# Quyans/SG-NeRF

Measured on AMD Instinct MI355X. Metric: rays/sec + ms/frame, 800×800×64 samples, ScanNet scene, 1/2/4/8 GPU, higher is better.
Workload: dtype f32 (3xf16 split MFMA, fp32 accumulate); 1 GPU; synth-room 800x800 rays x SR=64 samples, D=400, K=8, P=26, 1200000 neural points (BASELINE config 2, 1 frame per rank per step); rays_per_frame=640000, SR=64, K=8, D=400, points=1200000, parallelism=frame-sharded x1, outputs=rgb, ray mask, background transmission, coarse_point_opacity [R, SR]

## Files before the change

### sg-nerf_amd/csrc/mlp_x3.hip

```cpp
#include <cstdio>
#include <cstdlib>
#include <algorithm>
#include <cmath>
#include <utility>
#include <vector>

#include "agg_device.h"
#include "x3_split.h"

namespace sgn {
namespace {
namespace x3 {

constexpr int NW16 = 8, TPB16 = NW16 * 64;
constexpr int PAIR = 2048;
constexpr int NSLOT = 2;
constexpr int PD = 2;
constexpr size_t PROJ_BYTES_PER_POINT = HID * 4;
struct XL {
    int ks, tp, np, kc;
    uint32_t off;
};
__host__ __device__ constexpr int nch(XL l) { return (l.ks + l.kc - 1) / l.kc; }
__host__ __device__ constexpr int nk(XL l, int c) { return l.ks - c * l.kc < l.kc ? l.ks - c * l.kc : l.kc; }

template <class Net>
struct Sched {
    static constexpr int layer_chunks(int l) { return Net::L[l].np * nch(Net::L[l]); }
    static constexpr int base(int l) { return l == 0 ? 0 : base(l - 1) + layer_chunks(l - 1); }
    static constexpr int total() { return base(Net::NL); }
    static constexpr int idx(int l, int p, int c) { return base(l) + p * nch(Net::L[l]) + c; }
    static constexpr int cl(int n, int l = 0) { return (l + 1 >= Net::NL || n < base(l + 1)) ? l : cl(n, l + 1); }
    static constexpr int cp(int n) { return (n - base(cl(n))) / nch(Net::L[cl(n)]); }
    static constexpr int cc(int n) { return (n - base(cl(n))) % nch(Net::L[cl(n)]); }
    static constexpr uint32_t off(int n) {
        return Net::L[cl(n)].off +
               (uint32_t)((cp(n) * Net::L[cl(n)].ks + cc(n) * Net::L[cl(n)].kc) * Net::L[cl(n)].tp) * PAIR;
    }
    static constexpr int pairs(int n) { return nk(Net::L[cl(n)], cc(n)) * Net::L[cl(n)].tp; }
};

__device__ __forceinline__ X3Pair lrelu_split8(const float (&a)[8], float inv) {
    float v[8];
#pragma unroll
    for (int j = 0; j < 8; ++j) v[j] = lrelu_x3(a[j] * inv);
    return split8_unit(v);
}

__device__ __forceinline__ void lds_dma_1k(const WBlob &wb, char *dst, int w, int lane, uint32_t soff) {
    asm volatile("" : "+s"(soff));
    __builtin_amdgcn_raw_ptr_buffer_load_lds(wb.rsrc, (__attribute__((address_space(3))) void *)(dst + w * 1024), 16,
                                             lane * 16 + w * 1024, soff, 0, 0);
}

template <class Net, int N, int NWv = NW16>
__device__ __forceinline__ void dma_chunk(const WBlob &wb, char *dst, int w, int lane) {
    using S = Sched<Net>;
    constexpr int nf = 2 * S::pairs(N);
    static_for<(nf + NWv - 1) / NWv>([&](auto jj) {
        constexpr int J = decltype(jj)::value;
        const int i = w + NWv * J;
        if (NWv * (J + 1) <= nf || i < nf)
            lds_dma_1k(wb, dst + NWv * J * 1024, w, lane, S::off(N) + (uint32_t)(NWv * J * 1024));
    });
}

template <class Net, int N, int J, int NWv = NW16>
__device__ __forceinline__ void dma_piece(const WBlob &wb, char *dst, int w, int lane) {
    using S = Sched<Net>;
    constexpr int nf = 2 * S::pairs(N);
    constexpr int PW = (nf + NWv - 1) / NWv;
    const int i = w * PW + J;
    if (nf % NWv == 0 || i < nf) {
        uint32_t soff = S::off(N) + (uint32_t)((J & ~3) * 1024);
        asm volatile("" : "+s"(soff));
        __builtin_amdgcn_raw_ptr_buffer_load_lds(wb.rsrc,
                                                 (__attribute__((address_space(3))) void *)(dst + (w * PW + (J & ~3)) * 1024),
                                                 16, lane * 16 + w * PW * 1024, soff, (J & 3) * 1024, 0);
    }
}
template <class Net, int N, int NWv = NW16>
constexpr int dma_pieces() { return (2 * Sched<Net>::pairs(N) + NWv - 1) / NWv; }

template <int VM = 0>
__device__ __forceinline__ void chunk_enter() {
    static_assert(VM >= 0 && VM < 64, "vmcnt range");
    if constexpr (VM == 0)
        asm volatile("s_waitcnt vmcnt(0)" ::: "memory");
    else
        __builtin_amdgcn_s_waitcnt((VM & 15) | (7 << 4) | (15 << 8) | ((VM >> 4) << 14));
    asm volatile("s_waitcnt lgkmcnt(0)" ::: "memory");
    __builtin_amdgcn_s_barrier();
}

struct NoHook {
    template <class C>
    __device__ void operator()(C) const {}
};
struct VmZero {
    static constexpr int vm(int) { return 0; }
};

constexpr uint32_t OFF16_W0B = 0;
constexpr uint32_t OFF16_W1 = OFF16_W0B + 32 * PAIR;
constexpr uint32_t OFF16_W2 = OFF16_W1 + 128 * PAIR;
constexpr uint32_t OFF16_W3 = OFF16_W2 + 144 * PAIR;
constexpr uint32_t OFF16_W0A = OFF16_W3 + 128 * PAIR;
constexpr uint32_t OFF16_WB = OFF16_W0A + 112 * PAIR;
constexpr uint32_t OFF16_C0 = OFF16_WB + 176 * PAIR;
constexpr uint32_t OFF16_C1 = OFF16_C0 + 72 * PAIR;
constexpr uint32_t OFF16_C2 = OFF16_C1 + 32 * PAIR;
constexpr uint32_t OFF16_F32 = OFF16_C2 + 32 * PAIR;
constexpr int Y_B0 = 0, Y_B1 = 256, Y_B2 = 512, Y_B3 = 768, Y_WA = 1024, Y_BB = 1280, Y_BA = 1536, Y_INV = 1537;
constexpr int Y_CB0 = Y_INV + 8 + 3, Y_CB1 = Y_CB0 + 128, Y_CB2 = Y_CB1 + 128, Y_CW3 = Y_CB2 + 128, Y_CB3 = Y_CW3 + 384;
constexpr int N_Y32 = Y_CB3 + 4;
constexpr size_t BLOB_BYTES_ALL = OFF16_F32 + (size_t)N_Y32 * 4;
__host__ __device__ constexpr size_t blob_bytes_sg(int) { return BLOB_BYTES_ALL; }
static_assert(N_Y32 % 4 == 0, "fp32 section in 16-B units");

constexpr int NWR = 4;
struct NetR16T {
    static constexpr int NW = NWR, SP = 16;
    static constexpr int KC = SP / 16;
    static constexpr int NL = 4;
    static constexpr XL L[NL] = {{2, 16, 1, KC, OFF16_W0B}, {8, 16, 1, KC, OFF16_W1}, {9, 16, 1, KC, OFF16_W2},
                                 {8, 8, 2, 2 * KC, OFF16_W3}};
};
template <int KB>
struct NetR16SGT {
    static constexpr int NW = NetR16T::NW, SP = NetR16T::SP, KC = NetR16T::KC;
    static constexpr int NL = 5;
    static constexpr XL L[NL] = {{2, 16, 1, KC, OFF16_W0B}, {8, 16, 1, KC, OFF16_W1}, {KB, 16, 1, KC, OFF16_WB},
                                 {9, 16, 1, KC, OFF16_W2}, {8, 8, 2, 2 * KC, OFF16_W3}};
};
struct NetProj16 {
    static constexpr int NW = NW16, SP = 32;
    static constexpr int NL = 1;
    static constexpr XL L[NL] = {{7, 16, 1, 2, OFF16_W0A}};
};
constexpr int NWC = 8, SPC = 32, KCC = SPC / 8;
struct NetColor16 {
    static constexpr int NW = NWC, SP = SPC;
    static constexpr int NL = 3;
    static constexpr XL L[NL] = {{9, 8, 1, KCC, OFF16_C0}, {4, 8, 1, KCC, OFF16_C1}, {4, 8, 1, KCC, OFF16_C2}};
};
static_assert(Sched<NetR16T>::total() == 27, "16x16 row stream");
static_assert(Sched<NetColor16>::total() == 5 && Sched<NetColor16>::pairs(2) == 8, "16x16 colour stream");

__device__ __forceinline__ f32x4 mfma16(h8 a, h8 b, f32x4 c) {
    return __builtin_amdgcn_mfma_f32_16x16x32_f16(a, b, c, 0, 0, 0);
}

template <int NS>
struct X3S {
    X3Pair b[NS];
};

template <class Net, int L, bool TRANS = false, class Vm = VmZero, int P = 0, int AOFF = 0, bool PIPE = false,
          int NS, int NA, class InFn, class PostFn = NoHook, class EndFn = NoHook, class MidFn = NoHook>
__device__ __forceinline__ void run_layer_ns(const WBlob &wb, char *lds, int &slot, int w, int lane,
                                             f32x4 (&acc)[NS][NA], InFn &&in, PostFn &&post = PostFn{},
                                             EndFn &&end = EndFn{}, MidFn &&mid = MidFn{}) {
    constexpr XL ly = Net::L[L];
    constexpr int TP = ly.tp;
    static_assert((TP == 16 || TP == 8) && P < ly.np, "passes of 16 or 8 output tiles");
    static_assert(AOFF + TP <= NA, "accumulator view");
    X3S<NS> Bn;
    if constexpr (PIPE) Bn = in(std::integral_constant<int, 0>{});
    static_for<nch(ly)>([&](auto cc) {
        constexpr int C = decltype(cc)::value;
        constexpr int N = Sched<Net>::idx(L, P, C), NN = (N + 1) % Sched<Net>::total();
        constexpr int NWv = Net::NW, SLOTv = Net::SP * PAIR;
        static_assert(nk(ly, C) * TP <= Net::SP, "chunk larger than a ring slot");
        chunk_enter<Vm::vm(C)>();
        post(cc);
        const char *sl = lds + slot * SLOTv;
        char *dnext = lds + (slot ^ 1) * SLOTv;
        constexpr int NF = nk(ly, C) * TP;
        constexpr int PW = dma_pieces<Net, NN, NWv>();
        auto frag = [&](int f, int part) { return *(const h8 *)(sl + (2 * f + part) * 1024 + lane * 16); };
        h8 fh[PD], fl[PD];
#pragma unroll
        for (int f = 0; f < PD; ++f) {
            fh[f] = frag(f, 0);
            fl[f] = frag(f, 1);
        }
        __builtin_amdgcn_sched_group_barrier(0x100, 2 * PD, 0);
        static_for<nk(ly, C)>([&](auto kk) {
            constexpr int KK = decltype(kk)::value;
            constexpr int KS = C * ly.kc + KK;
            if constexpr (NS > 1 && KK > 0 && !PIPE) __builtin_amdgcn_sched_barrier(0);
            X3S<NS> B;
            if constexpr (PIPE) B = Bn;
            else B = in(std::integral_constant<int, KS>{});
            static_for<TP>([&](auto tt) {
                constexpr int t = decltype(tt)::value, F = KK * TP + t;
                const h8 Ah = fh[F % PD], Al = fl[F % PD];
                if constexpr (F + PD < NF) {
                    fh[F % PD] = frag(F + PD, 0);
                    fl[F % PD] = frag(F + PD, 1);
                }
#pragma unroll
                for (int s = 0; s < NS; ++s) {
                    f32x4 &c = acc[s][AOFF + t];
                    if constexpr (TRANS) {
                        c = mfma16(B.b[s].hi, Al, c);
                        c = mfma16(B.b[s].lo, Ah, c);
                        c = mfma16(B.b[s].hi, Ah, c);
                    } else {
                        c = mfma16(Al, B.b[s].hi, c);
                        c = mfma16(Ah, B.b[s].lo, c);
                        c = mfma16(Ah, B.b[s].hi, c);
                    }
                }
                constexpr int NSP = NF / 2 > 0 ? NF / 2 : 1;
                if constexpr (F < NSP) {
                    static_for<(F + 1) * PW / NSP - F * PW / NSP>([&](auto jj) {
                        dma_piece<Net, NN, F * PW / NSP + decltype(jj)::value, NWv>(wb, dnext, w, lane);
                    });
                }
                mid(std::integral_constant<int, (C * ly.kc + KK) * TP + t>{});
                if constexpr (PIPE && t == TP / 2 - 1 && KS + 1 < ly.ks)
                    Bn = in(std::integral_constant<int, (KS + 1 < ly.ks ? KS + 1 : KS)>{});
                if constexpr (NS == 1) {
                    __builtin_amdgcn_sched_group_barrier(0x008, 1, 0);
                    __builtin_amdgcn_sched_group_barrier(0x100, 1, 0);
                    __builtin_amdgcn_sched_group_barrier(0x008, 1, 0);
                    __builtin_amdgcn_sched_group_barrier(0x100, 1, 0);
                    __builtin_amdgcn_sched_group_barrier(0x008, 1, 0);
                } else {
                    __builtin_amdgcn_sched_group_barrier(0x008, 3 * NS / 2, 0);
                    __builtin_amdgcn_sched_group_barrier(0x100, 1, 0);
                    __builtin_amdgcn_sched_group_barrier(0x008, 3 * NS - 3 * NS / 2, 0);
                    __builtin_amdgcn_sched_group_barrier(0x100, 1, 0);
                }
            });
        });
        __builtin_amdgcn_sched_barrier(0);
        end(cc);
        slot ^= 1;
        __builtin_amdgcn_sched_barrier(0);
    });
}

template <class Net, int L, bool TRANS = false, class Vm = VmZero, int P = 0, class InFn,
          class PostFn = NoHook, class EndFn = NoHook, class MidFn = NoHook>
__device__ __forceinline__ void run_layer16(const WBlob &wb, char *lds, int &slot, int w, int lane,
                                            f32x4 (&acc)[Net::L[L].tp], InFn &&in, PostFn &&post = PostFn{},
                                            EndFn &&end = EndFn{}, MidFn &&mid = MidFn{}) {
    constexpr int TP = Net::L[L].tp;
    run_layer_ns<Net, L, TRANS, Vm, P, 0>(wb, lds, slot, w, lane, reinterpret_cast<f32x4(&)[1][TP]>(acc),
                                          [&](auto k) { return X3S<1>{{in(k)}}; }, post, end, mid);
}

struct Proj16Args {
    const float *emb;
    int64_t n;
    const void *blob;
    float *proj;
    const float *xyz, *color, *dir, *conf;
    float *rec;
    const int32_t *idx;
    const int64_t *n_dev;
};
constexpr int REC16_FLOATS = 16;
constexpr int Y_LDS_OFF = NSLOT * NetProj16::SP * PAIR;
constexpr int PROJ16_LDS = Y_LDS_OFF + N_Y32 * 4;

__global__ __launch_bounds__(TPB16, 1) void k_point_proj16(Proj16Args a) {
    __shared__ __attribute__((aligned(16))) char lds[PROJ16_LDS];
    const int lane = threadIdx.x & 63, g = lane >> 4;
    const int w = __builtin_amdgcn_readfirstlane(threadIdx.x >> 6);
    const WBlob wb = make_blob(a.blob, BLOB_BYTES_ALL);
    {
        const float *src = (const float *)((const char *)a.blob + OFF16_F32);
        float *dst = (float *)(lds + Y_LDS_OFF);
        for (int i = threadIdx.x; i < N_Y32; i += TPB16) dst[i] = src[i];
    }
    __syncthreads();
    int slot = 0;
    dma_chunk<NetProj16, 0, NW16>(wb, lds, w, lane);
    const int64_t n = a.idx ? min(*a.n_dev, a.n) : a.n;
    const int64_t ntile = (n + 16 * NW16 - 1) / (16 * NW16);
    for (int64_t tile = blockIdx.x; tile < ntile; tile += gridDim.x) {
        int lz = 0;
        asm volatile("" : "+s"(lz));
        const float *Yl = (const float *)(lds + lz + Y_LDS_OFF);
        const int64_t j = tile * (16 * NW16) + w * 16 + (lane & 15);
        const bool ok = j < n;
        const int64_t p = a.idx ? (ok ? (int64_t)a.idx[j] : 0) : j;
        float f8[8];
        {
            const f32x4 *e4 = (const f32x4 *)(a.emb + (ok ? p : 0) * 32 + 8 * g);
            const f32x4 u0 = e4[0], u1 = e4[1];
            f8[0] = u0[0]; f8[1] = u0[1]; f8[2] = u0[2]; f8[3] = u0[3];
            f8[4] = u1[0]; f8[5] = u1[1]; f8[6] = u1[2]; f8[7] = u1[3];
        }
        f32x4 acc[16];
#pragma unroll
        for (int t = 0; t < 16; ++t) acc[t] = *(const f32x4 *)(Yl + Y_B0 + 16 * t + 4 * g);
        auto in = [&](auto k) {
            constexpr int S = decltype(k)::value;
            float v[8];
            if constexpr (S == 0) {
#pragma unroll
                for (int j = 0; j < 8; ++j) v[j] = f8[j];
            } else {
                static_for<4>([&](auto jp) {
                    constexpr int q = 8 * (S - 1) + 2 * decltype(jp)::value, dl = q / 6, f = (q % 6) / 2;
                    float sv, cv;
                    sincos_f<f>(f8[dl], sv, cv);
                    v[2 * decltype(jp)::value] = sv;
                    v[2 * decltype(jp)::value + 1] = cv;
                });
            }
            return split8_unit(v);
        };
        f32x4 q{};
        {
            const float *src = g == 0 ? a.xyz : g == 1 ? a.color : a.dir;
            const int64_t pc = ok ? p : 0;
            if (g < 3) q = f32x4{src[pc * 3], src[pc * 3 + 1], src[pc * 3 + 2], g == 0 ? a.conf[pc] : 0.f};
        }
        run_layer16<NetProj16, 0>(wb, lds + lz, slot, w, lane, acc, in);
        if (ok) {
            float *dst = a.proj + p * HID + 4 * g;
#pragma unroll
            for (int t = 0; t < 16; ++t) *(f32x4 *)(dst + 16 * t) = acc[t];
            *(f32x4 *)(a.rec + p * REC16_FLOATS + 4 * g) = q;
        }
    }
    asm volatile("s_waitcnt vmcnt(0)" ::: "memory");
}

constexpr int WG16_SAMPLES = NWR * 2;
constexpr int TPBR = NWR * 64;
constexpr int YR_OFF = NSLOT * NetR16T::SP * PAIR;
constexpr int YT16_OFF = YR_OFF + N_Y32 * 4;
constexpr int ROWS16_LDS = YT16_OFF + 2 * 16 * 20 * 4;
static_assert(2 * ROWS16_LDS <= 163840, "LDS budget (16x16 rows, two workgroups per CU)");

template <bool PERS, bool ROT = false>
struct Rec16 {
    float p[3], col[3], dir[3], cf, l[3], v[3];
    float pp[PERS ? 3 : 1], pl[PERS ? 3 : 1];
    float R[ROT ? 9 : 1];
};
constexpr int REC16_LOADS = 9;
template <bool PERS, bool ROT = false>
__device__ __forceinline__ Rec16<PERS, ROT> load_rec16(const AggArgs &a, const RowIdx &ix) {
    Rec16<PERS, ROT> r;
    const bool v = ix.sval;
    const int pid = ix.pid, s = ix.s, ray = ix.ray;
    const bool m = v && pid >= 0;
    const float *dummy = (const float *)a.blob;
    const f32x4 *rp = (const f32x4 *)(m ? a.rec + (int64_t)pid * REC16_FLOATS : dummy);
    const float *lp = v ? a.samp_locw + (int64_t)s * 3 : dummy;
    const float *vp = v ? (ROT ? a.samp_v + (int64_t)s * 3 : a.raydir + (int64_t)ray * 3) : dummy;
    const f32x4 q0 = rp[0], q1 = rp[1], q2 = rp[2];
    if constexpr (ROT) {
        const float *Rp = m ? a.prot + (int64_t)pid * 9 : dummy;
#pragma unroll
        for (int c = 0; c < 9; ++c) r.R[c] = Rp[c];
    }
    float l3[3], v3[3];
#pragma unroll
    for (int c = 0; c < 3; ++c) {
        l3[c] = lp[c];
        v3[c] = vp[c];
    }
#pragma unroll
    for (int c = 0; c < 3; ++c) {
        r.p[c] = m ? q0[c] : 0.f;
        r.col[c] = m ? q1[c] : 0.f;
        r.dir[c] = m ? q2[c] : 0.f;
        r.l[c] = v ? l3[c] : 0.f;
        r.v[c] = v ? v3[c] : 0.f;
        if constexpr (PERS) {
            r.pp[c] = m ? a.pers[(int64_t)pid * 3 + c] : 0.f;
            r.pl[c] = v ? a.samp_pers[(int64_t)s * 3 + c] : 0.f;
        }
    }
    r.cf = m ? q0[3] : 0.f;
    return r;
}
template <int NS>
struct VmL3P0 {
    static constexpr int vm(int c) { return c == 1 ? NS * (REC16_LOADS + 1) : 0; }
};
template <int NS>
struct VmL0 {
    static constexpr int vm(int c) { return c == 0 ? 16 * NS : 0; }
};

constexpr int PAIR_TPB = 1024, PAIR_NW = PAIR_TPB / 64;
__global__ __launch_bounds__(PAIR_TPB) void k_pair_slots(const int32_t *__restrict__ counters,
                                                         const int32_t *__restrict__ work,
                                                         const int32_t *__restrict__ nnb, int32_t item0,
                                                         int32_t n_items, int32_t pair, int32_t *__restrict__ rows,
                                                         int4 *__restrict__ slots, int32_t *__restrict__ slot_n) {
    __shared__ int wc[PAIR_NW][9], nt[9];
    __shared__ int16_t blist[9][PAIR_TPB];
    __shared__ int ss[PAIR_TPB];
    __shared__ int8_t sc[PAIR_TPB];
    __shared__ int wl[PAIR_NW], sbase;
    const int tid = threadIdx.x, lane = tid & 63, wv = tid >> 6;
    const int end = min(counters[1], item0 + n_items);
    for (int rel0 = blockIdx.x * PAIR_TPB; item0 + rel0 < end; rel0 += gridDim.x * PAIR_TPB) {
        __syncthreads();
        const int item = item0 + rel0 + tid;
        const bool ok = item < end;
        const int s = ok ? work[item] : 0;
        const int c = ok ? min(max(nnb[s], 1), 8) : 0;
        ss[tid] = s;
        sc[tid] = (int8_t)c;
        const uint64_t below = (1ull << lane) - 1ull;
        int rank = 0;
#pragma unroll
        for (int b = 1; b <= 8; ++b) {
            const uint64_t m = __ballot(c == b);
            if (c == b) rank = __popcll(m & below);
            if (lane == 0) wc[wv][b] = __popcll(m);
        }
// ... 107 lines not shown
    }
    float xp, yp, zp, xl, yl, zl;
    if constexpr (PERS) {
        xp = rc.pp[0]; yp = rc.pp[1]; zp = rc.pp[2];
        xl = rc.pl[0]; yl = rc.pl[1]; zl = rc.pl[2];
    } else {
        cam.pers(rc.p[0], rc.p[1], rc.p[2], xp, yp, zp);
        cam.pers(rc.l[0], rc.l[1], rc.l[2], xl, yl, zl);
    }
    o.d[3] = m ? __fsub_rn(__fmul_rn(xp, zp), __fmul_rn(xl, zl)) : 0.f;
    o.d[4] = m ? __fsub_rn(__fmul_rn(yp, zp), __fmul_rn(yl, zl)) : 0.f;
    o.d[5] = m ? __fsub_rn(zp, zl) : 0.f;
    float w = 0.f;
    if (m) {
        const float n2 = __fadd_rn(__fadd_rn(__fmul_rn(dwx, dwx), __fmul_rn(dwy, dwy)), __fmul_rn(dwz, dwz));
        w = 1.f / fmaxf(sqrtf(n2), 1e-6f);
    }
    float wsum;
    if (waveB) {
        const float wb0 = isA ? 0.f : w;
        const int rb0 = __builtin_bit_cast(int, wb0);
        const int r1 = __builtin_amdgcn_mov_dpp(rb0, 0x39, 0xF, 0xF, true);
        const int r2 = __builtin_amdgcn_mov_dpp(rb0, 0x4E, 0xF, 0xF, true);
        const int r3 = __builtin_amdgcn_mov_dpp(rb0, 0x93, 0xF, 0xF, true);
        const int rot = nA > 4 ? nA - 4 : 0;
        const float wbs = __builtin_bit_cast(float, rot == 0 ? rb0 : rot == 1 ? r1 : rot == 2 ? r2 : r3);
        const float wsa = dpp_sum8(isA ? w : 0.f), wsb = dpp_sum8(wbs);
        wsum = isA ? wsa : wsb;
    } else {
        wsum = dpp_sum8(w);
    }
    w = w / fmaxf(wsum, 1e-8f);
    o.wn = w;
    o.wgt = w * fminf(fmaxf(rc.cf, 1e-4f), 1.f);
    return o;
}

struct PeRow {
    float lo, hi, shi;
};
__device__ __forceinline__ PeRow pe_row16(const float (&d)[6], int g) {
    PeRow r;
    r.lo = g == 0 ? d[0] : g == 1 ? d[1] : g == 2 ? d[2] : d[3];
    r.hi = (g & 1) ? d[5] : d[4];
    r.shi = g >= 2 ? 2.f : 1.f;
    return r;
}
template <int C>
__device__ __forceinline__ float pe_arg16(const PeRow &r) {
    if constexpr (C < 5) return r.lo * (float)(1 << C);
    else if constexpr (C == 7) return r.hi * 16.f;
    else return r.hi * (r.shi * (float)(1 << (2 * (C - 5))));
}
template <int S>
__device__ __forceinline__ X3Pair pe_dists16_k(const PeRow &r) {
    float x[4], u[8];
    static_for<4>([&](auto cc) { x[decltype(cc)::value] = pe_arg16<4 * S + decltype(cc)::value>(r); });
    const float m = fmaxf(fmaxf(__builtin_fabsf(x[0]), __builtin_fabsf(x[1])), fmaxf(__builtin_fabsf(x[2]), __builtin_fabsf(x[3])));
    if (__builtin_expect(__ballot(!(m < 1048576.f)) != 0, 0)) {
#pragma unroll
        for (int q = 0; q < 4; ++q) sincosf(x[q], &u[2 * q], &u[2 * q + 1]);
    } else {
#pragma unroll
        for (int q = 0; q < 4; ++q) sincos_acc_fast(x[q], u[2 * q], u[2 * q + 1]);
    }
    return split8_unit(u);
}

struct Epi16 {
    float wsa[4], wsb[4];
    float ap[4];
    float fsv[4];
    float *fs_dst;
    bool fs_have;
};

struct Tiles {
    int first, end, step;
};
__device__ __forceinline__ Tiles grid_tiles(int ntiles) { return Tiles{(int)blockIdx.x, ntiles, (int)gridDim.x}; }

template <int KB, bool PERS, bool SAVE = false, int NS = 1, bool ROT = false>
__global__ __launch_bounds__(TPBR, NS == 1 ? 8 / NWR : 1) void k_rows16(AggArgs a) {
    using Net = std::conditional_t<(KB > 0), NetR16SGT<KB>, NetR16T>;
    constexpr int LB = 2, L2 = KB ? 3 : 2, L3 = KB ? 4 : 3;
    constexpr int NBP = KB > 8 ? KB - 8 : 0;
    constexpr int WGS = WG16_SAMPLES * NS;
    __shared__ __attribute__((aligned(16))) char lds[ROWS16_LDS];
    const int lane = threadIdx.x & 63;
    const int g = lane >> 4, r = lane & 15, kk = lane & 7, sc = r >> 3;
    const int w = __builtin_amdgcn_readfirstlane(threadIdx.x >> 6);
    const int nslots = a.slot_n[0];
    const Cam cam = load_cam(a.campos, a.rot);
    const WBlob wb = make_blob(a.blob, BLOB_BYTES_ALL);
    const float *proj = (const float *)a.proj;
    {
        const float *src = (const float *)((const char *)a.blob + OFF16_F32);
        float *dst = (float *)(lds + YR_OFF);
        for (int i = threadIdx.x; i < N_Y32; i += TPBR) dst[i] = src[i];
        {
            float *yt = (float *)(lds + YT16_OFF);
            for (int i = threadIdx.x; i < 512; i += TPBR) {
                const int which = i >> 8, u = i & 255, t = u >> 4, rr = u & 15;
                yt[which * 320 + rr * 20 + t] = src[(which ? Y_WA : Y_B3) + 16 * t + rr];
            }
        }
    }
    __syncthreads();
    int slot = 0;
    dma_chunk<Net, 0, NWR>(wb, lds, w, lane);
    const Tiles xt = grid_tiles((nslots + WGS - 1) / WGS);
    RowIdx nx[NS];
    Rec16<PERS, ROT> rnext[NS];
#pragma unroll
    for (int q = 0; q < NS; ++q) {
        nx[q] = row_index16(a, xt.first * WGS + w * 2 * NS + 2 * q + sc, nslots, kk);
        rnext[q] = load_rec16<PERS, ROT>(a, nx[q]);
    }
    auto load_p = [&](int pid, f32x4 (&dst)[16]) {
        const float *src = proj + (int64_t)(pid < 0 ? 0 : pid) * HID + 4 * g;
#pragma unroll
        for (int t = 0; t < 16; ++t) dst[t] = *(const f32x4 *)(src + 16 * t);
    };
    f32x4 accA[NS][16], accB[NS][16];
#pragma unroll
    for (int q = 0; q < NS; ++q) load_p(nx[q].pid, pick<(KB > 0)>(accB[q], accA[q]));

    auto epi_begin = [&](Epi16 &e, const char *ldsi, float wgt, int nA, int nB, int2 ce, bool ok) {
        const float inv3 = ((const float *)(ldsi + YR_OFF))[Y_INV + 3];
#pragma unroll
        for (int i = 0; i < 4; ++i) {
            const float wi = __builtin_bit_cast(float, __builtin_amdgcn_ds_bpermute((4 * g + i) * 4, __builtin_bit_cast(int, wgt)));
            const bool inA = 4 * (g & 1) + i < nA;
            const float ws = wi * inv3;
            e.wsa[i] = inA ? ws : 0.f;
            e.wsb[i] = inA ? 0.f : ws;
            e.ap[i] = 0.f;
        }
        e.fs_have = ((g & 1) ? nB > 0 : nA > 0) && ok;
        e.fs_dst = (float *)a.fs + (int64_t)((uint32_t)((g & 1) ? ce.y : ce.x) & 0x0FFFFFFFu) * HID + r;
    };
    auto epi_step = [&](Epi16 &e, const char *ldsi, const f32x4 (&ac)[16], auto tc) {
        constexpr int T = decltype(tc)::value;
        const float wau = ((const float *)(ldsi + YT16_OFF))[320 + r * 20 + T];
        float fa = 0.f, fb = 0.f;
#pragma unroll
        for (int i = 0; i < 4; ++i) {
            const float hv = lrelu_x3(ac[T][i]);
            e.ap[i] = __builtin_fmaf(wau, hv, e.ap[i]);
            fa = __builtin_fmaf(e.wsa[i], hv, fa);
            fb = __builtin_fmaf(e.wsb[i], hv, fb);
        }
        permlane16_swap(fa, fb);
        e.fsv[T & 3] = fa + fb;
        if constexpr ((T & 3) == 3) {
            if (e.fs_have) {
#pragma unroll
                for (int u = 0; u < 4; ++u) e.fs_dst[16 * (T - 3 + u)] = e.fsv[u];
            }
        }
    };
    auto epi_end = [&](Epi16 &e, const char *ldsi, int nA, int nB, int s_ix) {
        const float ba = ((const float *)(ldsi + YR_OFF))[Y_BA];
        const float sc3 = __builtin_bit_cast(float, 0x7F000000 - __builtin_bit_cast(int, ((const float *)(ldsi + YR_OFF))[Y_INV + 3]));
        float xr[4];
#pragma unroll
        for (int i = 0; i < 4; ++i) {
            float x = dpp_sum8(e.ap[i]);
            x += __builtin_bit_cast(float, __builtin_amdgcn_mov_dpp(__builtin_bit_cast(int, x), 0x128, 0xF, 0xF, true));
            xr[i] = x;
        }
        const int q4 = r & 3;
        const float spm = softplus((q4 == 0 ? xr[0] : q4 == 1 ? xr[1] : q4 == 2 ? xr[2] : xr[3]) + ba - 1.f);
        const int spi = __builtin_bit_cast(int, spm);
        const float sp4[4] = {__builtin_bit_cast(float, __builtin_amdgcn_mov_dpp(spi, 0x00, 0xF, 0xF, true)),
                              __builtin_bit_cast(float, __builtin_amdgcn_mov_dpp(spi, 0x55, 0xF, 0xF, true)),
                              __builtin_bit_cast(float, __builtin_amdgcn_mov_dpp(spi, 0xAA, 0xF, 0xF, true)),
                              __builtin_bit_cast(float, __builtin_amdgcn_mov_dpp(spi, 0xFF, 0xF, 0xF, true))};
        float asa = 0.f, asb = 0.f;
#pragma unroll
        for (int i = 0; i < 4; ++i) {
            asa = __builtin_fmaf(e.wsa[i], sp4[i], asa);
            asb = __builtin_fmaf(e.wsb[i], sp4[i], asb);
        }
        permlane16_swap(asa, asb);
        const float as = (asa + asb) * sc3;
        const int s_of = __builtin_amdgcn_ds_bpermute((8 * (g >> 1) + ((g & 1) ? (nA > 4 ? nA : 4) : 0)) * 4, s_ix);
        if (r == 0 && ((g & 1) ? nB > 0 : nA > 0)) a.feat[(int64_t)s_of * 4 + 0] = as;
    };

    for (int tile = xt.first; tile < xt.end; tile += xt.step) {
        const int base = tile * WGS;
        int lz = 0;
        asm volatile("" : "+s"(lz));
        char *ldsi = lds + lz;
        const float *Yl = (const float *)(ldsi + YR_OFF);
        RowIdx ix[NS];
        Row16 rw[NS];
        int nslot[NS], nA[NS], nB[NS];
        uint64_t mrowA[NS], mrowB[NS];
        int64_t vrow[NS];
        X3Pair ext[NS];
        const int hsh = 8 * (g >> 1);
#pragma unroll
        for (int q = 0; q < NS; ++q) {
            const int hslot = base + w * 2 * NS + 2 * q + sc;
            nslot[q] = tile + xt.step < xt.end ? hslot + xt.step * WGS : nslots;
            ix[q] = nx[q];
            const bool m = ix[q].pid >= 0;
            const Rec16<PERS, ROT> rc = rnext[q];
            mrowA[q] = __ballot(ix[q].sval && ix[q].a);
            mrowB[q] = __ballot(ix[q].sval && !ix[q].a);
            const int nA0 = __popc((uint32_t)mrowA[q] & 0xFFu), nA1 = __popc(((uint32_t)mrowA[q] >> 8) & 0xFFu);
            const bool waveB = (mrowB[q] & 0xFFFFull) != 0;
            rw[q] = row_math16<PERS, ROT>(cam, rc, m, ix[q].a, sc ? nA1 : nA0, waveB);
            nA[q] = __popcll((mrowA[q] >> hsh) & 0xFFull);
            nB[q] = __popcll((mrowB[q] >> hsh) & 0xFFull);
            vrow[q] = -1;
            if (SAVE && ix[q].sval && m) {
                const int e = a.rows[(int64_t)hslot * 8 + kk];
                vrow[q] = a.row_off ? (int64_t)a.row_off[e >> 3] + (e & 7) : pidx_of(a, e);
            }
            if ((a.blend || a.wnorm) && ix[q].sval) {
                const int64_t v = pidx_of(a, a.rows[(int64_t)hslot * 8 + kk]);
                if (a.blend && g == 0) a.blend[v] = rw[q].wgt;
                if (a.wnorm && g == 1) a.wnorm[v] = rw[q].wn;
            }
            {
                const bool e = g == 0 && m;
                float u[8], pd[3] = {rc.dir[0], rc.dir[1], rc.dir[2]};
                if constexpr (ROT) rot3(rc.R, pd[0], pd[1], pd[2], pd[0], pd[1], pd[2]);
                u[0] = e ? rc.col[0] : 0.f; u[1] = e ? rc.col[1] : 0.f; u[2] = e ? rc.col[2] : 0.f;
                u[3] = e ? __fsub_rn(pd[0], rc.v[0]) : 0.f;
                u[4] = e ? __fsub_rn(pd[1], rc.v[1]) : 0.f;
                u[5] = e ? __fsub_rn(pd[2], rc.v[2]) : 0.f;
                u[6] = e ? __fadd_rn(__fadd_rn(__fmul_rn(pd[0], rc.v[0]), __fmul_rn(pd[1], rc.v[1])),
                                     __fmul_rn(pd[2], rc.v[2])) : 0.f;
                u[7] = 0.f;
                ext[q] = split8_unit(u);
            }
        }
        auto chain_k = [&](int q, const f32x4 (&ac)[16], float inv, auto kc, float *zsave = nullptr) {
            constexpr int S = decltype(kc)::value;
            float v[8];
#pragma unroll
            for (int j = 0; j < 8; ++j) v[j] = ac[2 * S + (j >> 2)][j & 3];
            if constexpr (SAVE) {
                if (zsave && vrow[q] >= 0) {
                    float *zr = zsave + vrow[q] * HID + 4 * g;
                    *(f32x4 *)(zr + 32 * S) = f32x4{v[0] * inv, v[1] * inv, v[2] * inv, v[3] * inv};
                    *(f32x4 *)(zr + 32 * S + 16) = f32x4{v[4] * inv, v[5] * inv, v[6] * inv, v[7] * inv};
                }
            }
            return lrelu_split8(v, inv);
        };
        auto bias_init = [&](f32x4 (&ac)[16], int yb) {
#pragma unroll
            for (int t = 0; t < 16; ++t) ac[t] = *(const f32x4 *)(Yl + yb + 16 * t + 4 * g);
        };
        {
            PeRow pr[NS];
#pragma unroll
            for (int q = 0; q < NS; ++q) {
                pr[q] = pe_row16(rw[q].d, g);
                if constexpr (KB > 0) {
#pragma unroll
                    for (int t = 0; t < 16; ++t) accA[q][t] = accB[q][t];
                }
            }
            run_layer_ns<Net, 0, false, std::conditional_t<SAVE, VmZero, VmL0<NS>>, 0, 0, !SAVE>(
                wb, ldsi, slot, w, lane, accA, [&](auto k) {
                    X3S<NS> o;
#pragma unroll
                    for (int q = 0; q < NS; ++q) o.b[q] = pe_dists16_k<decltype(k)::value>(pr[q]);
                    return o;
                }, NoHook{});
        }
        const float inv0 = Yl[Y_INV + 0], inv1 = Yl[Y_INV + 1], inv2 = Yl[Y_INV + 2], inv7 = Yl[Y_INV + 7];
#pragma unroll
        for (int q = 0; q < NS; ++q) bias_init(accB[q], Y_B1);
        int v_next[NS];
        run_layer_ns<Net, 1, false, VmZero, 0, 0, !SAVE>(wb, ldsi, slot, w, lane, accB, [&](auto k) {
            X3S<NS> o;
#pragma unroll
            for (int q = 0; q < NS; ++q) o.b[q] = chain_k(q, accA[q], inv0, k, a.z1);
            return o;
        }, [&](auto c) {
            if constexpr (decltype(c)::value == 0) {
#pragma unroll
                for (int q = 0; q < NS; ++q) v_next[q] = nslot[q] < nslots ? a.rows[(int64_t)nslot[q] * 8 + kk] : -1;
            }
        });
        if constexpr (KB > 0) {
            X3Pair bpv[NS][NBP > 0 ? NBP : 1];
            if constexpr (NBP > 0) {
#pragma unroll
                for (int q = 0; q < NS; ++q) {
                    const float *src = a.bpnet32 + (int64_t)(ix[q].pid >= 0 ? ix[q].pid : 0) * (NBP * 32) + 8 * g;
#pragma unroll
                    for (int j = 0; j < NBP; ++j) {
                        const f32x4 u0 = *(const f32x4 *)(src + 32 * j), u1 = *(const f32x4 *)(src + 32 * j + 4);
                        const float v[8] = {u0[0], u0[1], u0[2], u0[3], u1[0], u1[1], u1[2], u1[3]};
                        bpv[q][j] = split8_unit(v);
                    }
                }
            }
#pragma unroll
            for (int q = 0; q < NS; ++q) bias_init(accA[q], Y_BB);
            run_layer_ns<Net, LB>(wb, ldsi, slot, w, lane, accA, [&](auto k) {
                constexpr int K = decltype(k)::value;
                X3S<NS> o;
#pragma unroll
                for (int q = 0; q < NS; ++q) {
                    if constexpr (K < 8) o.b[q] = chain_k(q, accB[q], inv1, k, a.z2);
                    else o.b[q] = bpv[q][K - 8];
                }
                return o;
            }, NoHook{});
        }
        auto &in2 = pick<(KB > 0)>(accA, accB);
        auto &acc2 = pick<(KB > 0)>(accB, accA);
        const float inv_in2 = KB > 0 ? inv7 : inv1;
#pragma unroll
        for (int q = 0; q < NS; ++q) bias_init(acc2[q], Y_B2);
        run_layer_ns<Net, L2, false, VmZero, 0, 0, !SAVE>(wb, ldsi, slot, w, lane, acc2, [&](auto k) {
            constexpr int K = decltype(k)::value;
            X3S<NS> o;
#pragma unroll
            for (int q = 0; q < NS; ++q) {
                if constexpr (K < 8) o.b[q] = chain_k(q, in2[q], inv_in2, k, KB > 0 ? a.zb : a.z2);
                else o.b[q] = ext[q];
            }
            return o;
        }, [&](auto c) {
            constexpr int C = decltype(c)::value;
            if constexpr (C == 0) {
#pragma unroll
                for (int q = 0; q < NS; ++q) {
                    nx[q].sval = v_next[q] >= 0;
                    nx[q].s = nx[q].sval ? v_next[q] >> 3 : 0;
                    nx[q].a = (v_next[q] & 7) == kk;
                    nx[q].pid = nx[q].sval ? a.pidx[pidx_of(a, v_next[q])] : -1;
                    nx[q].ray = nx[q].sval ? a.samp_ray[nx[q].s] : 0;
                }
            }
        });
        auto &acc = in2;
        {
            const f32x4 *yb = (const f32x4 *)(ldsi + YT16_OFF + r * 80);
#pragma unroll
            for (int j = 0; j < 4; ++j) {
                const f32x4 b4 = yb[j];
#pragma unroll
                for (int q = 0; q < NS; ++q)
#pragma unroll
                    for (int i = 0; i < 4; ++i) acc[q][4 * j + i] = f32x4{b4[i], b4[i], b4[i], b4[i]};
            }
        }
        int2 ce[NS];
        int eslot[NS];
#pragma unroll
        for (int q = 0; q < NS; ++q) {
            ce[q] = make_int2(0, 0);
            eslot[q] = base + w * 2 * NS + 2 * q + (g >> 1);
        }
        auto first_chunk_loads = [&](auto c) {
            if constexpr (decltype(c)::value == 0) {
#pragma unroll
                for (int q = 0; q < NS; ++q) {
                    rnext[q] = load_rec16<PERS, ROT>(a, nx[q]);
                    ce[q] = *(const int2 *)(a.slots + (eslot[q] < nslots ? eslot[q] : 0));
                }
            }
        };
        Epi16 e[NS];
        {
            X3Pair in3[NS][8];
            run_layer_ns<Net, L3, true, std::conditional_t<SAVE, VmZero, VmL3P0<NS>>, 0, 0, !SAVE>(
                wb, ldsi, slot, w, lane, acc, [&](auto k) {
                    constexpr int K = decltype(k)::value;
                    X3S<NS> o;
#pragma unroll
                    for (int q = 0; q < NS; ++q) {
                        in3[q][K] = chain_k(q, acc2[q], inv2, k, a.z3);
                        o.b[q] = in3[q][K];
                    }
                    return o;
                }, NoHook{}, first_chunk_loads);
#pragma unroll
            for (int q = 0; q < NS; ++q) epi_begin(e[q], ldsi, rw[q].wgt, nA[q], nB[q], ce[q], eslot[q] < nslots);
            run_layer_ns<Net, L3, true, VmZero, 1, 8>(wb, ldsi, slot, w, lane, acc, [&](auto k) {
                X3S<NS> o;
#pragma unroll
                for (int q = 0; q < NS; ++q) o.b[q] = in3[q][decltype(k)::value];
                return o;
            }, NoHook{}, NoHook{}, [&](auto f) {
                constexpr int F = decltype(f)::value;
                if constexpr ((F & 7) == 7) {
#pragma unroll
                    for (int q = 0; q < NS; ++q) epi_step(e[q], ldsi, acc[q], std::integral_constant<int, F / 8>{});
                }
            });
        }
#pragma unroll
        for (int q = 0; q < NS; ++q) {
            asm volatile("" : "+v"(nx[q].s), "+v"(nx[q].pid), "+v"(nx[q].ray));
#pragma unroll
            for (int c = 0; c < 3; ++c) {
                asm volatile("" : "+v"(rnext[q].p[c]), "+v"(rnext[q].col[c]), "+v"(rnext[q].dir[c]), "+v"(rnext[q].l[c]),
                             "+v"(rnext[q].v[c]));
                if constexpr (PERS) asm volatile("" : "+v"(rnext[q].pp[c]), "+v"(rnext[q].pl[c]));
            }
            asm volatile("" : "+v"(rnext[q].cf));
            if constexpr (ROT) {
#pragma unroll
                for (int c = 0; c < 9; ++c) asm volatile("" : "+v"(rnext[q].R[c]));
            }
        }
        {
            constexpr int NE = 8, PPE = 16 / NE;
            static_for<NE>([&](auto tc) {
                constexpr int J = decltype(tc)::value;
#pragma unroll
                for (int q = 0; q < NS; ++q) {
                    const float *psrc = proj + (int64_t)(nx[q].pid < 0 ? 0 : nx[q].pid) * HID + 4 * g;
#pragma unroll
                    for (int u = 0; u < PPE; ++u) acc2[q][PPE * J + u] = *(const f32x4 *)(psrc + 16 * (PPE * J + u));
                    epi_step(e[q], ldsi, acc[q], std::integral_constant<int, (16 - NE) + J>{});
                }
            });
#pragma unroll
            for (int q = 0; q < NS; ++q) epi_end(e[q], ldsi, nA[q], nB[q], ix[q].s);
        }
    }
    asm volatile("s_waitcnt vmcnt(0)" ::: "memory");
}

int perm16(int p) { return 16 * ((p & 7) >> 2) + 4 * (p >> 3) + (p & 3); }
int col_chain16(int ks, int p) { return 32 * ks + perm16(p); }
int col_l2_16(int ks, int p) { return ks < 8 ? col_chain16(ks, p) : (p < 7 ? 256 + p : -1); }
int col_l0b16(int s, int p) {
    const int g = p >> 3, c = 4 * s + ((p & 7) >> 1);
    int comp, f;
    if (c < 5) {
        comp = g;
        f = c;
    } else {
        comp = 4 + (g & 1);
        f = c == 5 ? (g >= 2) : c == 6 ? 2 + (g >= 2) : 4;
        if (c == 7 && g >= 2) return -1;
    }
    return 224 + 2 * (5 * comp + f) + (p & 1);
}
int col_proj16(int s, int p) { return s == 0 ? p : 32 + 48 * (p >> 3) + 8 * (s - 1) + (p & 7); }
int col_bp16(int ks, int p) { return ks < 8 ? col_chain16(ks, p) : 256 + 32 * (ks - 8) + p; }
int col_c016(int ks, int p) {
    if (ks < 8) return 32 * ks + p;
    const int g = p >> 3, f = (p & 7) >> 1;
    return g < 3 ? 256 + ((p & 1) ? 12 : 0) + 4 * g + f : -1;
}

template <typename ColFn>
void pack_pairs16(_Float16 *dst, const float *W, int n_out, int n_in, int KS, int shift, ColFn col, int NT = 16,
                  int NP = 1) {
    const float sc = ldexpf(1.f, shift);
    const int TPP = NT / NP;
    for (int t = 0; t < NT; ++t)
        for (int ks = 0; ks < KS; ++ks) {
            const size_t f = ((size_t)(t / TPP) * KS + ks) * TPP + t % TPP;
            for (int lane = 0; lane < 64; ++lane)
                for (int e = 0; e < 8; ++e) {
                    const int row = 16 * t + (lane & 15);
                    const int c = col(ks, 8 * (lane >> 4) + e);
                    const float v = (row < n_out && c >= 0 && c < n_in) ? W[(size_t)row * n_in + c] * sc : 0.f;
                    const _Float16 hi = (_Float16)v;
                    const _Float16 lo = (_Float16)(v - (float)hi);
                    dst[((2 * f) * 64 + lane) * 8 + e] = hi;
                    dst[((2 * f + 1) * 64 + lane) * 8 + e] = lo;
                }
        }
}

enum Y32Kind { YK_ZERO = 0, YK_W = 1, YK_B = 2, YK_BS = 3, YK_INV = 4, YK_ONE = 5, YK_WINV = 6, YK_BS_OR_B = 7 };
template <class Pairs, class F32>
void layout_blob16(int ksb, int bpnet_dim, Pairs &&pairs, F32 &&f32) {
    pairs(OFF16_W0B, 0, 256, 284, 2, col_l0b16, 16, 1);
    pairs(OFF16_W1, 1, 256, 256, 8, col_chain16, 16, 1);
    pairs(OFF16_W2, 2, 256, 263, 9, col_l2_16, 16, 1);
    pairs(OFF16_W3, 3, 256, 256, 8, col_chain16, 16, 2);
    pairs(OFF16_W0A, 0, 256, 284, 7, col_proj16, 16, 1);
    for (int u = 0; u < HID; ++u) {
        f32(Y_B0 + u, YK_BS, 0, u);
        f32(Y_B1 + u, YK_BS, 1, u);
        f32(Y_B2 + u, YK_BS, 2, u);
        f32(Y_B3 + u, YK_BS, 3, u);
        f32(Y_WA + u, YK_WINV, 4, u);
    }
    f32(Y_BA, YK_B, 4, 0);
    const int li[7] = {0, 1, 2, 3, 5, 6, 7};
    for (int i = 0; i < 7; ++i) f32(Y_INV + i, YK_INV, li[i], 0);
    f32(Y_INV + 7, ksb > 0 ? YK_INV : YK_ONE, 9, 0);
    if (ksb > 0) {
        pairs(OFF16_WB, 9, 256, 256 + bpnet_dim, 8 + bpnet_dim / 32, col_bp16, 16, 1);
        for (int u = 0; u < HID; ++u) f32(Y_BB + u, YK_BS, 9, u);
    }
    pairs(OFF16_C0, 5, 128, 280, 9, col_c016, 8, 1);
    pairs(OFF16_C1, 6, 128, 128, 4, col_chain16, 8, 1);
    pairs(OFF16_C2, 7, 128, 128, 4, col_chain16, 8, 1);
    for (int u = 0; u < 128; ++u) {
        f32(Y_CB0 + u, YK_BS, 5, u);
        f32(Y_CB1 + u, YK_BS, 6, u);
        f32(Y_CB2 + u, YK_BS, 7, u);
        for (int c = 0; c < 3; ++c) f32(Y_CW3 + 128 * c + u, YK_W, 8, c * 128 + u);
    }
    for (int c = 0; c < 3; ++c) f32(Y_CB3 + c, YK_B, 8, c);
}

void pack_blob16(int ksb, int bpnet_dim, const float *const *w, const float *const *b, const int *s, int sb,
                 uint8_t *blob) {
    auto shift = [&](int L) { return L == 9 ? sb : s[L]; };
    float *Y = (float *)(blob + OFF16_F32);
    layout_blob16(ksb, bpnet_dim,
                  [&](uint32_t off, int L, int n_out, int n_in, int KS, auto col, int NT, int NP) {
                      pack_pairs16((_Float16 *)(blob + off), w[L], n_out, n_in, KS, shift(L), col, NT, NP);
                  },
                  [&](int yi, int kind, int L, int e) {
                      float v = 0.f;
                      switch (kind) {
                          case YK_W: v = w[L][e]; break;
                          case YK_B: v = b[L][e]; break;
                          case YK_BS: v = b[L][e] * ldexpf(1.f, shift(L)); break;
                          case YK_INV: v = ldexpf(1.f, -shift(L)); break;
                          case YK_ONE: v = 1.f; break;
                          case YK_WINV: v = w[L][e] * ldexpf(1.f, -shift(3)); break;
                          default: break;
                      }
                      Y[yi] = v;
                  });
}

void index_blob16(int ksb, int bpnet_dim, int32_t *i16, size_t n16, int32_t *i32, size_t n32) {
    for (size_t i = 0; i < n16; ++i) i16[i] = -1;
    for (size_t i = 0; i < n32; ++i) i32[i] = 0;
    layout_blob16(ksb, bpnet_dim,
                  [&](uint32_t off, int L, int n_out, int n_in, int KS, auto col, int NT, int NP) {
                      const int TPP = NT / NP;
                      int32_t *dst = i16 + off / 2;
                      for (int t = 0; t < NT; ++t)
                          for (int ks = 0; ks < KS; ++ks) {
                              const size_t f = ((size_t)(t / TPP) * KS + ks) * TPP + t % TPP;
                              for (int lane = 0; lane < 64; ++lane)
                                  for (int e = 0; e < 8; ++e) {
                                      const int row = 16 * t + (lane & 15);
                                      const int c = col(ks, 8 * (lane >> 4) + e);
                                      const bool ok = row < n_out && c >= 0 && c < n_in;
                                      const int32_t code = ok ? (L << 20) | (row * n_in + c) : -1;
                                      dst[((2 * f) * 64 + lane) * 8 + e] = code;
                                      dst[((2 * f + 1) * 64 + lane) * 8 + e] = ok ? code | (1 << 30) : -1;
                                  }
                          }
                  },
                  [&](int yi, int kind, int L, int e) { i32[yi] = (kind << 26) | (L << 20) | e; });
}
struct ColorArgs {
    const int32_t *counters, *work, *samp_ray;
    const float *raydir;
    const void *blob;
    const float *fs;
    float *feat;
    int32_t *range_flag;
    int32_t item0, n_items;
    const float *viewdir;
};
constexpr int YC_OFF = NSLOT * SPC * PAIR, TPBC = NWC * 64;
constexpr int COL16_LDS = YC_OFF + N_Y32 * 4;
static_assert(COL16_LDS <= 163840, "LDS budget (colour, one workgroup per CU)");

template <bool ROT = false>
__global__ __launch_bounds__(TPBC, 1) void k_color16(ColorArgs a) {
    __shared__ __attribute__((aligned(16))) char lds[COL16_LDS];
    const int lane = threadIdx.x & 63;
    const int g = lane >> 4, r = lane & 15;
    const int w = __builtin_amdgcn_readfirstlane(threadIdx.x >> 6);
    const int nwork = a.counters[1];
    const int end = min(nwork, a.item0 + a.n_items);
    const WBlob wb = make_blob(a.blob, BLOB_BYTES_ALL);
    {
        const float *src = (const float *)((const char *)a.blob + OFF16_F32);
        float *dst = (float *)(lds + YC_OFF);
        for (int i = threadIdx.x; i < N_Y32; i += TPBC) dst[i] = src[i];
    }
    __syncthreads();
    int slot = 0;
    dma_chunk<NetColor16, 0, NWC>(wb, lds, w, lane);
    f32x4 fr[16];
    float vd[3];
    int sn = 0, rn = 0;
    auto load_q = [&](auto qc, int item) {
        constexpr int Q = decltype(qc)::value;
        const bool ok = item < end;
        const f32x4 *row = (const f32x4 *)(a.fs + (int64_t)(ok ? item - a.item0 : 0) * HID + 8 * g) + 16 * Q;
        f32x4 t0, t1, t2, t3;
        asm volatile("global_load_dwordx4 %0, %1, off" : "=v"(t0) : "v"(row));
        asm volatile("global_load_dwordx4 %0, %1, off offset:16" : "=v"(t1) : "v"(row));
        asm volatile("global_load_dwordx4 %0, %1, off offset:128" : "=v"(t2) : "v"(row));
        asm volatile("global_load_dwordx4 %0, %1, off offset:144" : "=v"(t3) : "v"(row));
        fr[4 * Q] = t0;
        fr[4 * Q + 1] = t1;
        fr[4 * Q + 2] = t2;
        fr[4 * Q + 3] = t3;
    };
    auto load_sid = [&](int item) { sn = item < end ? a.work[item] : 0; };
    auto load_ray = [&]() { rn = a.samp_ray[sn]; };
    auto load_dir = [&]() {
#pragma unroll
        for (int c = 0; c < 3; ++c) vd[c] = ROT ? a.viewdir[(int64_t)sn * 3 + c] : a.raydir[(int64_t)rn * 3 + c];
    };
    {
        const int item = a.item0 + blockIdx.x * (16 * NWC) + w * 16 + r;
        load_sid(item);
        load_q(std::integral_constant<int, 0>{}, item);
        load_q(std::integral_constant<int, 1>{}, item);
        load_q(std::integral_constant<int, 2>{}, item);
        asm volatile("s_waitcnt vmcnt(0)" ::: "memory");
    }
    load_ray();
    for (int base = a.item0 + blockIdx.x * (16 * NWC); base < end; base += gridDim.x * (16 * NWC)) {
        int lz = 0;
        asm volatile("" : "+s"(lz));
        char *ldsi = lds + lz;
        const float *Yl = (const float *)(ldsi + YC_OFF);
        const int item = base + w * 16 + r;
        const bool sval = item < end;
        const int s = sn;
        auto bias = [&](f32x4 (&ac)[8], int yb) {
#pragma unroll
            for (int t = 0; t < 8; ++t) ac[t] = *(const f32x4 *)(Yl + yb + 16 * t + 4 * g);
        };
        auto chain = [&](const f32x4 (&ac)[8], float inv, auto kc) {
            constexpr int S = decltype(kc)::value;
            float v[8];
#pragma unroll
            for (int j = 0; j < 8; ++j) v[j] = ac[2 * S + (j >> 2)][j & 3];
// ... 330 lines not shown
```

Baseline: 25.39 million rays/s.

## Split layer-2 extra input columns into a single-fragment MFMA chunk

Layer 2's ninth K-step, which carried the 7 extra per-sample inputs through the 3xf16 split-pair path, is replaced by one dedicated chunk of 16 single f16 MFMAs. Hi/lo parts of the weights and inputs are arranged across lane groups so each product needs one MFMA instead of a pair. For NS=1 the chunk streams through the existing double-buffered weight DMA. For NS=2 it is preloaded once into extra LDS. This is meant to cut MFMA and weight-streaming work for the extra columns, at the cost of more LDS for NS=2, a changed blob layout, and possibly slightly different split precision.

```diff
diff --git a/sg-nerf_amd/csrc/mlp_x3.hip b/sg-nerf_amd/csrc/mlp_x3.hip
--- a/sg-nerf_amd/csrc/mlp_x3.hip
+++ b/sg-nerf_amd/csrc/mlp_x3.hip
@@ -104,7 +104,9 @@
 constexpr uint32_t OFF16_W0B = 0;
 constexpr uint32_t OFF16_W1 = OFF16_W0B + 32 * PAIR;
 constexpr uint32_t OFF16_W2 = OFF16_W1 + 128 * PAIR;
-constexpr uint32_t OFF16_W3 = OFF16_W2 + 144 * PAIR;
+constexpr uint32_t OFF16_X2 = OFF16_W2 + 128 * PAIR;
+constexpr int X2_BYTES = 16 * 1024;
+constexpr uint32_t OFF16_W3 = OFF16_X2 + X2_BYTES;
 constexpr uint32_t OFF16_W0A = OFF16_W3 + 128 * PAIR;
 constexpr uint32_t OFF16_WB = OFF16_W0A + 112 * PAIR;
 constexpr uint32_t OFF16_C0 = OFF16_WB + 176 * PAIR;
@@ -119,19 +121,20 @@
 static_assert(N_Y32 % 4 == 0, "fp32 section in 16-B units");
 
 constexpr int NWR = 4;
+template <int XC>
 struct NetR16T {
     static constexpr int NW = NWR, SP = 16;
     static constexpr int KC = SP / 16;
-    static constexpr int NL = 4;
-    static constexpr XL L[NL] = {{2, 16, 1, KC, OFF16_W0B}, {8, 16, 1, KC, OFF16_W1}, {9, 16, 1, KC, OFF16_W2},
-                                 {8, 8, 2, 2 * KC, OFF16_W3}};
-};
-template <int KB>
+    static constexpr int NL = 5;
+    static constexpr XL L[NL] = {{2, 16, 1, KC, OFF16_W0B}, {8, 16, 1, KC, OFF16_W1}, {8, 16, 1, KC, OFF16_W2},
+                                 {XC, 8, 1, 1, OFF16_X2}, {8, 8, 2, 2 * KC, OFF16_W3}};
+};
+template <int KB, int XC>
 struct NetR16SGT {
-    static constexpr int NW = NetR16T::NW, SP = NetR16T::SP, KC = NetR16T::KC;
-    static constexpr int NL = 5;
+    static constexpr int NW = NetR16T<XC>::NW, SP = NetR16T<XC>::SP, KC = NetR16T<XC>::KC;
+    static constexpr int NL = 6;
     static constexpr XL L[NL] = {{2, 16, 1, KC, OFF16_W0B}, {8, 16, 1, KC, OFF16_W1}, {KB, 16, 1, KC, OFF16_WB},
-                                 {9, 16, 1, KC, OFF16_W2}, {8, 8, 2, 2 * KC, OFF16_W3}};
+                                 {8, 16, 1, KC, OFF16_W2}, {XC, 8, 1, 1, OFF16_X2}, {8, 8, 2, 2 * KC, OFF16_W3}};
 };
 struct NetProj16 {
     static constexpr int NW = NW16, SP = 32;
@@ -144,7 +147,10 @@
     static constexpr int NL = 3;
     static constexpr XL L[NL] = {{9, 8, 1, KCC, OFF16_C0}, {4, 8, 1, KCC, OFF16_C1}, {4, 8, 1, KCC, OFF16_C2}};
 };
-static_assert(Sched<NetR16T>::total() == 27, "16x16 row stream");
+static_assert(Sched<NetR16T<0>>::total() == 26 && Sched<NetR16T<1>>::total() == 27, "16x16 row stream");
+static_assert(Sched<NetR16T<1>>::pairs(18) == 8 && Sched<NetR16T<1>>::off(18) == OFF16_X2 &&
+                  Sched<NetR16T<1>>::off(19) == OFF16_W3 && Sched<NetR16T<0>>::off(18) == OFF16_W3,
+              "block3.0's extras: a chunk of 8 pair slots in the NS = 1 stream only");
 static_assert(Sched<NetColor16>::total() == 5 && Sched<NetColor16>::pairs(2) == 8, "16x16 colour stream");
 
 __device__ __forceinline__ f32x4 mfma16(h8 a, h8 b, f32x4 c) {
@@ -253,6 +259,37 @@
                                           [&](auto k) { return X3S<1>{{in(k)}}; }, post, end, mid);
 }
 
+template <int NS, int NA>
+__device__ __forceinline__ void ext_mfmas(const char *frags, int lane, f32x4 (&acc)[NS][NA], const h8 (&ext)[NS]) {
+    constexpr int QD = 2 * PD;
+    auto frag = [&](int t) { return *(const h8 *)(frags + t * 1024 + lane * 16); };
+    h8 fx[QD];
+#pragma unroll
+    for (int f = 0; f < QD; ++f) fx[f] = frag(f);
+    static_for<16>([&](auto tt) {
+        constexpr int t = decltype(tt)::value;
+        const h8 A = fx[t % QD];
+        if constexpr (t + QD < 16) fx[t % QD] = frag(t + QD);
+#pragma unroll
+        for (int s = 0; s < NS; ++s) acc[s][t] = mfma16(A, ext[s], acc[s][t]);
+    });
+}
+
+template <class Net, int L, int NS, int NA>
+__device__ __forceinline__ void run_ext_chunk(const WBlob &wb, char *lds, int &slot, int w, int lane,
+                                              f32x4 (&acc)[NS][NA], const h8 (&ext)[NS]) {
+    constexpr int N = Sched<Net>::idx(L, 0, 0), NN = (N + 1) % Sched<Net>::total();
+    constexpr int NWv = Net::NW, SLOTv = Net::SP * PAIR;
+    static_assert(nch(Net::L[L]) == 1 && Sched<Net>::pairs(N) * PAIR == X2_BYTES, "one chunk of 16 single fragments");
+    chunk_enter<0>();
+    char *dnext = lds + (slot ^ 1) * SLOTv;
+    static_for<dma_pieces<Net, NN, NWv>()>([&](auto jj) { dma_piece<Net, NN, decltype(jj)::value, NWv>(wb, dnext, w, lane); });
+    ext_mfmas(lds + slot * SLOTv, lane, acc, ext);
+    __builtin_amdgcn_sched_barrier(0);
+    slot ^= 1;
+    __builtin_amdgcn_sched_barrier(0);
+}
+
 struct Proj16Args {
     const float *emb;
     int64_t n;
@@ -335,10 +372,13 @@
 
 constexpr int WG16_SAMPLES = NWR * 2;
 constexpr int TPBR = NWR * 64;
-constexpr int YR_OFF = NSLOT * NetR16T::SP * PAIR;
+constexpr int YR_OFF = NSLOT * NetR16T<0>::SP * PAIR;
 constexpr int YT16_OFF = YR_OFF + N_Y32 * 4;
 constexpr int ROWS16_LDS = YT16_OFF + 2 * 16 * 20 * 4;
+constexpr int XR_OFF = ROWS16_LDS;
 static_assert(2 * ROWS16_LDS <= 163840, "LDS budget (16x16 rows, two workgroups per CU)");
+static_assert(XR_OFF % 16 == 0, "16-B fragment reads");
+static_assert(XR_OFF + X2_BYTES <= 163840, "LDS budget (16x16 rows, NS = 2)");
 
 template <bool PERS, bool ROT = false>
 struct Rec16 {
@@ -612,11 +652,12 @@
 
 template <int KB, bool PERS, bool SAVE = false, int NS = 1, bool ROT = false>
 __global__ __launch_bounds__(TPBR, NS == 1 ? 8 / NWR : 1) void k_rows16(AggArgs a) {
-    using Net = std::conditional_t<(KB > 0), NetR16SGT<KB>, NetR16T>;
-    constexpr int LB = 2, L2 = KB ? 3 : 2, L3 = KB ? 4 : 3;
+    constexpr int XC = NS == 1;
+    using Net = std::conditional_t<(KB > 0), NetR16SGT<KB, XC>, NetR16T<XC>>;
+    constexpr int LB = 2, L2 = KB ? 3 : 2, LX = L2 + 1, L3 = L2 + 2;
     constexpr int NBP = KB > 8 ? KB - 8 : 0;
     constexpr int WGS = WG16_SAMPLES * NS;
-    __shared__ __attribute__((aligned(16))) char lds[ROWS16_LDS];
+    __shared__ __attribute__((aligned(16))) char lds[ROWS16_LDS + (XC ? 0 : X2_BYTES)];
     const int lane = threadIdx.x & 63;
     const int g = lane >> 4, r = lane & 15, kk = lane & 7, sc = r >> 3;
     const int w = __builtin_amdgcn_readfirstlane(threadIdx.x >> 6);
@@ -635,6 +676,12 @@
                 yt[which * 320 + rr * 20 + t] = src[(which ? Y_WA : Y_B3) + 16 * t + rr];
             }
         }
+        if constexpr (!XC) {
+#pragma unroll
+            for (int j = 0; j < X2_BYTES / (NWR * 1024); ++j)
+                lds_dma_1k(wb, lds + XR_OFF + j * NWR * 1024, w, lane, OFF16_X2 + (uint32_t)(j * NWR * 1024));
+            asm volatile("s_waitcnt vmcnt(0)" ::: "memory");
+        }
     }
     __syncthreads();
     int slot = 0;
@@ -730,7 +777,7 @@
         int nslot[NS], nA[NS], nB[NS];
         uint64_t mrowA[NS], mrowB[NS];
         int64_t vrow[NS];
-        X3Pair ext[NS];
+        h8 ext[NS];
         const int hsh = 8 * (g >> 1);
 #pragma unroll
         for (int q = 0; q < NS; ++q) {
@@ -757,7 +804,7 @@
                 if (a.wnorm && g == 1) a.wnorm[v] = rw[q].wn;
             }
             {
-                const bool e = g == 0 && m;
+                const bool e = g < 3 && m;
                 float u[8], pd[3] = {rc.dir[0], rc.dir[1], rc.dir[2]};
                 if constexpr (ROT) rot3(rc.R, pd[0], pd[1], pd[2], pd[0], pd[1], pd[2]);
                 u[0] = e ? rc.col[0] : 0.f; u[1] = e ? rc.col[1] : 0.f; u[2] = e ? rc.col[2] : 0.f;
@@ -767,7 +814,8 @@
                 u[6] = e ? __fadd_rn(__fadd_rn(__fmul_rn(pd[0], rc.v[0]), __fmul_rn(pd[1], rc.v[1])),
                                      __fmul_rn(pd[2], rc.v[2])) : 0.f;
                 u[7] = 0.f;
-                ext[q] = split8_unit(u);
+                const X3Pair us = split8_unit(u);
+                ext[q] = g == 1 ? us.lo : us.hi;
             }
         }
         auto chain_k = [&](int q, const f32x4 (&ac)[16], float inv, auto kc, float *zsave = nullptr) {
@@ -854,13 +902,9 @@
 #pragma unroll
         for (int q = 0; q < NS; ++q) bias_init(acc2[q], Y_B2);
         run_layer_ns<Net, L2, false, VmZero, 0, 0, !SAVE>(wb, ldsi, slot, w, lane, acc2, [&](auto k) {
-            constexpr int K = decltype(k)::value;
             X3S<NS> o;
 #pragma unroll
-            for (int q = 0; q < NS; ++q) {
-                if constexpr (K < 8) o.b[q] = chain_k(q, in2[q], inv_in2, k, KB > 0 ? a.zb : a.z2);
-                else o.b[q] = ext[q];
-            }
+            for (int q = 0; q < NS; ++q) o.b[q] = chain_k(q, in2[q], inv_in2, k, KB > 0 ? a.zb : a.z2);
             return o;
         }, [&](auto c) {
             constexpr int C = decltype(c)::value;
@@ -875,6 +919,12 @@
                 }
             }
         });
+        if constexpr (XC) run_ext_chunk<Net, LX>(wb, ldsi, slot, w, lane, acc2, ext);
+        else {
+            __builtin_amdgcn_sched_barrier(0);
+            ext_mfmas(ldsi + XR_OFF, lane, acc2, ext);
+            __builtin_amdgcn_sched_barrier(0);
+        }
         auto &acc = in2;
         {
             const f32x4 *yb = (const f32x4 *)(ldsi + YT16_OFF + r * 80);
@@ -968,7 +1018,7 @@
 
 int perm16(int p) { return 16 * ((p & 7) >> 2) + 4 * (p >> 3) + (p & 3); }
 int col_chain16(int ks, int p) { return 32 * ks + perm16(p); }
-int col_l2_16(int ks, int p) { return ks < 8 ? col_chain16(ks, p) : (p < 7 ? 256 + p : -1); }
+int sel_x2_16(int lane, int e) { return ((lane >> 4) < 3 && e < 7) ? (256 + e) | (((lane >> 4) == 2) << 16) : -1; }
 int col_l0b16(int s, int p) {
     const int g = p >> 3, c = 4 * s + ((p & 7) >> 1);
     int comp, f;
@@ -1011,12 +1061,24 @@
         }
 }
 
+template <typename SelFn, typename Each>
+void singles16(int n_out, int n_in, int NT, SelFn sel, Each &&each) {
+    for (int t = 0; t < NT; ++t)
+        for (int lane = 0; lane < 64; ++lane)
+            for (int e = 0; e < 8; ++e) {
+                const int row = 16 * t + (lane & 15), sv = sel(lane, e), c = sv & 0xFFFF;
+                const bool ok = sv >= 0 && row < n_out && c < n_in;
+                each(((size_t)t * 64 + lane) * 8 + e, ok ? row * n_in + c : -1, ok ? sv >> 16 : 0);
+            }
+}
+
 enum Y32Kind { YK_ZERO = 0, YK_W = 1, YK_B = 2, YK_BS = 3, YK_INV = 4, YK_ONE = 5, YK_WINV = 6, YK_BS_OR_B = 7 };
-template <class Pairs, class F32>
-void layout_blob16(int ksb, int bpnet_dim, Pairs &&pairs, F32 &&f32) {
+template <class Pairs, class Singles, class F32>
+void layout_blob16(int ksb, int bpnet_dim, Pairs &&pairs, Singles &&singles, F32 &&f32) {
     pairs(OFF16_W0B, 0, 256, 284, 2, col_l0b16, 16, 1);
     pairs(OFF16_W1, 1, 256, 256, 8, col_chain16, 16, 1);
-    pairs(OFF16_W2, 2, 256, 263, 9, col_l2_16, 16, 1);
+    pairs(OFF16_W2, 2, 256, 263, 8, col_chain16, 16, 1);
+    singles(OFF16_X2, 2, 256, 263, 16, sel_x2_16);
     pairs(OFF16_W3, 3, 256, 256, 8, col_chain16, 16, 2);
     pairs(OFF16_W0A, 0, 256, 284, 7, col_proj16, 16, 1);
     for (int u = 0; u < HID; ++u) {
@@ -1053,6 +1115,15 @@
     layout_blob16(ksb, bpnet_dim,
                   [&](uint32_t off, int L, int n_out, int n_in, int KS, auto col, int NT, int NP) {
                       pack_pairs16((_Float16 *)(blob + off), w[L], n_out, n_in, KS, shift(L), col, NT, NP);
+                  },
+                  [&](uint32_t off, int L, int n_out, int n_in, int NT, auto sel) {
+                      _Float16 *dst = (_Float16 *)(blob + off);
+                      const float sc = ldexpf(1.f, shift(L));
+                      singles16(n_out, n_in, NT, sel, [&](size_t i, int el, int part) {
+                          const float v = el >= 0 ? w[L][el] * sc : 0.f;
+                          const _Float16 hi = (_Float16)v;
+                          dst[i] = part ? (_Float16)(v - (float)hi) : hi;
+                      });
                   },
                   [&](int yi, int kind, int L, int e) {
                       float v = 0.f;
@@ -1089,6 +1160,12 @@
                                       dst[((2 * f + 1) * 64 + lane) * 8 + e] = ok ? code | (1 << 30) : -1;
                                   }
                           }
+                  },
+                  [&](uint32_t off, int L, int n_out, int n_in, int NT, auto sel) {
+                      int32_t *dst = i16 + off / 2;
+                      singles16(n_out, n_in, NT, sel, [&](size_t i, int el, int part) {
+                          dst[i] = el >= 0 ? (L << 20) | el | (part ? 1 << 30 : 0) : -1;
+                      });
                   },
                   [&](int yi, int kind, int L, int e) { i32[yi] = (kind << 26) | (L << 20) | e; });
 }
```

Measured after the change: 25.45 million rays/s (median of 6 runs). Within noise of the previous version (+0.3%).
